# zhen6618/EPRecon

Hardware: AMD Instinct MI355X
Metric: fragments_per_sec (higher is better)
Workload: dtype f32

## Files before the change

### eprecon_amd/_lib.py

```python
import ctypes
import os

import torch

_HERE = os.path.dirname(os.path.abspath(__file__))
LIB_PATH = os.environ.get("EPRECON_LIB_PATH") or os.path.join(_HERE, "libeprecon_hip.so")

_c = ctypes
_vp, _i, _i64, _f, _sz = _c.c_void_p, _c.c_int, _c.c_int64, _c.c_float, _c.c_size_t

SIGNATURES = {
    "eprecon_abi_version": (_i, []),
    "eprecon_build_arch": (_c.c_char_p, []),
    "eprecon_back_project_workspace_bytes": (_sz, [_i64, _i, _i, _i, _i, _i, _i]),
    "eprecon_back_project_async": (_i, [_vp, _i64, _vp, _i, _f, _vp, _i, _vp, _i, _i, _i, _i, _i, _i,
                                        _vp, _vp, _vp, _vp, _vp, _vp, _vp, _vp, _sz, _vp]),
    "eprecon_back_project_call_async": (_i, [_vp, _vp]),
    "eprecon_back_project_call": (_i, [_vp, _i, _vp, _vp]),
    "eprecon_back_project_prepare_levels_async": (_i, [_vp, _i, _vp]),
    "eprecon_back_project_workspace_maps_offset": (_sz, [_i64, _i]),
    "eprecon_bp_levels": (_i, []),
    "eprecon_init_glue": (_i, []),
    "eprecon_profile_gather_kernel": (_c.c_char_p, []),
    "eprecon_hash_capacity": (_c.c_uint32, [_i64]),
# ... 72 lines not shown
    "eprecon_devoxelize_gate_tail_async": (_i, [_vp, _i, _vp, _vp, _i64, _i, _vp, _i, _i, _vp, _i, _vp, _i, _vp, _i, _vp, _i, _vp, _i,
                                                _i, _vp]),
    "eprecon_fbv_union_workspace_bytes": (_sz, [_i]),
    "eprecon_fbv_union_async": (_i, [_vp, _vp, _i64, _i, _vp, _vp, _i64, _i, _i, _i, _i, _i, _vp, _vp, _vp, _vp, _vp,
                                     _vp, _vp, _sz, _vp]),
    "eprecon_map_set_fragment": (_i, [_vp, _i]),
    "eprecon_map_stamps_async": (_i, [_vp, _vp, _vp, _i, _c.c_int32, _vp]),
    "eprecon_map_select_boundary_async": (_i, [_vp, _vp, _i, _i, _i, _vp, _vp]),
    "eprecon_map_pack_boundary_async": (_i, [_vp, _vp, _i64, _vp]),
    "eprecon_map_merge_boundary": (_i, [_vp, _vp, _i64, _vp, _i, _vp, _vp]),
    "eprecon_map_create": (_i, [_i, _c.POINTER(_vp)]),
    "eprecon_map_destroy": (_i, [_vp]),
    "eprecon_map_reset": (_i, [_vp]),
    "eprecon_map_size": (_i64, [_vp]),
    "eprecon_map_channels": (_i, [_vp]),
    "eprecon_map_export_async": (_i, [_vp, _vp, _vp, _vp]),
    "eprecon_map_import_async": (_i, [_vp, _vp, _vp, _i64, _vp]),
    "eprecon_map_crop_union": (_i, [_vp, _vp, _vp, _i64, _i, _i, _i, _i, _vp, _vp, _vp, _vp, _vp, _vp]),
    "eprecon_map_gather_async": (_i, [_vp, _vp, _i64, _i, _i, _f, _vp, _i, _vp]),
    "eprecon_map_update_async": (_i, [_vp, _vp, _i64, _vp, _i, _vp]),
    "eprecon_map_target_fuse": (_i, [_vp, _vp, _vp, _i, _vp, _vp, _i64, _vp, _vp]),
    "eprecon_gather_rows_async": (_i, [_vp, _i, _vp, _i64, _i, _f, _vp, _i, _vp]),
    "eprecon_tsdf_integrate_async": (_i, [_vp, _vp, _vp, _vp, _f, _vp, _i, _i, _i, _vp, _vp, _f, _f, _i, _vp, _vp]),
    "eprecon_gt_crop_async": (_i, [_vp, _vp]),
    "eprecon_label_volumes_workspace_bytes": (_sz, [_i64, _i64]),
    "eprecon_label_volumes": (_i, [_vp, _vp, _vp, _vp, _i64, _vp, _c.c_double, _vp, _vp, _vp, _vp, _vp, _sz, _vp]),
    "eprecon_label_fill_workspace_bytes": (_sz, [_i, _i, _i]),
    "eprecon_label_fill_async": (_i, [_vp, _vp, _vp, _vp, _sz, _vp]),
    "eprecon_marching_cubes_table": (_i, [_vp]),
    "eprecon_marching_cubes_workspace_bytes": (_sz, [_i, _i, _i]),
    "eprecon_marching_cubes_count": (_i, [_vp, _i, _i, _i, _f, _vp, _vp, _sz, _vp]),
    "eprecon_marching_cubes_emit_async": (_i, [_vp, _i, _i, _i, _f, _vp, _vp, _vp, _vp, _vp, _vp, _vp, _vp, _vp]),
    "eprecon_marching_cubes_count_masked": (_i, [_vp, _vp, _i, _i, _i, _f, _vp, _vp, _sz, _vp]),
    "eprecon_marching_cubes_emit_masked_async": (_i, [_vp, _vp, _i, _i, _i, _f, _vp, _vp, _vp, _vp, _vp, _vp, _vp, _vp, _vp]),
    "eprecon_render_depth_workspace_bytes": (_sz, [_i64]),
    "eprecon_render_depth_async": (_i, [_vp, _i64, _vp, _i64, _vp, _i, _i, _i, _f, _f, _f, _i, _vp, _i64, _vp, _sz, _vp]),
    "eprecon_render_visibility_workspace_bytes": (_sz, [_i64]),
    "eprecon_render_visibility_async": (_i, [_vp, _i64, _vp, _i64, _vp, _i, _i, _i, _f, _f, _f, _i, _vp, _i64, _vp, _sz, _vp]),
    "eprecon_render_resolve_async": (_i, [_vp, _vp, _i64, _vp, _i64, _vp, _i, _i, _i, _f, _vp, _vp, _vp, _vp, _c.c_int32, _vp, _vp,
                                          _c.c_int32, _vp, _vp, _c.c_double, _i, _i, _i, _vp, _vp]),
    "eprecon_depth_metrics_workspace_bytes": (_sz, [_i]),
    "eprecon_depth_metrics_async": (_i, [_vp, _vp, _i, _i64, _vp, _vp, _sz, _vp]),
    "eprecon_point_bounds_async": (_i, [_vp, _i64, _vp, _vp, _vp]),
    "eprecon_voxel_down_sample_workspace_bytes": (_sz, [_i64, _i64]),
    "eprecon_voxel_down_sample": (_i, [_vp, _i64, _vp, _c.c_double, _vp, _vp, _vp, _i64, _vp, _sz, _vp]),
    "eprecon_nn_search_workspace_bytes": (_sz, [_i64, _i64]),
    "eprecon_nn_search_async": (_i, [_vp, _i64, _vp, _i64, _vp, _c.c_double, _vp, _vp, _vp, _vp, _sz, _vp]),
    "eprecon_label_transfer_workspace_bytes": (_sz, [_vp, _i64]),
    "eprecon_label_bricks_async": (_i, [_vp, _vp, _vp, _i, _vp, _vp, _vp]),
    "eprecon_label_transfer_async": (_i, [_vp, _vp, _vp, _vp, _vp, _c.c_double, _vp, _i, _vp, _i64, _i, _vp, _vp, _vp, _vp, _vp, _sz,
                                          _vp]),
    "eprecon_instance_vote_async": (_i, [_vp, _vp, _i64, _i, _i, _vp, _vp, _vp, _sz, _vp]),
    "eprecon_pair_count_async": (_i, [_vp, _vp, _i64, _i, _i, _vp, _vp, _vp]),
    "eprecon_voxel_pair_count_async": (_i, [_vp, _vp, _vp, _vp, _vp, _vp, _vp, _c.c_double, _c.c_double, _f, _vp, _vp, _i, _i, _vp,
                                            _vp, _vp]),
    "eprecon_nearest_voxel_async": (_i, [_vp, _c.c_uint32, _vp, _i64, _vp, _i64, _i, _vp, _vp]),
    "eprecon_upsample2x_nhwc_async": (_i, [_vp, _vp, _i, _i, _i, _i, _vp]),
    "eprecon_decoder_keys_async": (_i, [_vp, _i, _vp, _i, _vp, _vp, _vp, _i64, _i, _vp, _vp, _vp]),
    "eprecon_decoder_query_side_async": (_i, [_vp, _vp]),
    "eprecon_panoptic_stats_async": (_i, [_vp, _i64, _vp, _vp, _i, _i64, _vp, _vp, _vp, _vp]),
    "eprecon_panoptic_assign_async": (_i, [_vp, _vp, _vp, _i64, _vp, _vp]),
    "eprecon_masked_attention_workspace_bytes": (_sz, [_i64, _i, _i, _i]),
    "eprecon_masked_attention_async": (_i, [_vp, _i, _i, _vp, _i, _vp, _i, _i64, _vp, _i, _vp, _i64, _i, _i, _i, _f, _vp, _vp, _sz, _vp]),
    "eprecon_profile_enable": (_i, [_i]),
    "eprecon_profile_gather_ms": (_f, []),
    "eprecon_profile_conv_arm": (_i, [_i, _i, _i, _i64]),
    "eprecon_profile_conv_ms": (_f, [_c.POINTER(_i64), _c.POINTER(_c.c_char_p)]),
    "eprecon_profile_conv_pairs": (_i64, []),
    "eprecon_mlp4x_supported": (_i, [_i, _i]),
    "eprecon_spvcnn_forward_workspace_bytes": (_sz, [_vp]),
    "eprecon_spvcnn_forward_async": (_i, [_vp, _vp]),
    "eprecon_spvcnn_geometry_workspace_bytes": (_sz, [_i64, _i64, _i64]),
    "eprecon_spvcnn_geometry_async": (_i, [_vp, _vp]),
    "eprecon_gru_stage_finish_workspace_bytes": (_sz, [_i64, _i64, _i64]),
    "eprecon_gru_stage_finish_async": (_i, [_vp, _vp]),
    "eprecon_bn2d_views_chunks": (_i, [_i64, _i]),
    "eprecon_bn2d_views_workspace_bytes": (_sz, [_i, _i64, _i]),
    "eprecon_bn2d_views_stats_async": (_i, [_vp, _i, _i64, _i, _vp, _vp, _f, _vp, _vp, _sz, _vp]),
    "eprecon_bn2d_views_apply_async": (_i, [_vp, _i, _i64, _i, _vp, _i, _vp, _vp, _vp]),
    "eprecon_dwconv2d_nhwc_async": (_i, [_vp, _i, _i, _i, _i, _vp, _i, _i, _vp, _i, _i, _vp, _vp]),
    "eprecon_mlp4x_async": (_i, [_vp, _vp]),
    "eprecon_profile_conv_executed_pairs": (_i64, []),
    "eprecon_profile_last_conv_kernel": (_c.c_char_p, []),
    "eprecon_profile_mark_async": (_i, [_i, _vp]),
    "eprecon_conv_desc_workspace_bytes": (_sz, [_vp]),
    "eprecon_sparsify_workspace_bytes": (_sz, [_i64]),
    "eprecon_sparsify_async": (_i, [_vp, _i, _f, _vp, _vp, _vp, _i, _vp, _i, _i, _i, _i64, _i, _vp, _vp, _vp, _vp, _vp, _vp, _vp,
                                    _sz, _vp]),
    "eprecon_grid_rank_async": (_i, [_vp, _i64, _i, _i, _i, _i, _vp, _vp]),
    "eprecon_conv_pack_weight_floats": (_sz, [_i, _i, _i]),
    "eprecon_conv_pack_weight_async": (_i, [_vp, _i, _i, _i, _vp, _vp]),
    "eprecon_conv_pack_weight16_floats": (_sz, [_i, _i, _i]),
    "eprecon_conv_pack_weight16_async": (_i, [_vp, _i, _i, _i, _vp, _vp]),
    "eprecon_conv_pack_many_async": (_i, [_vp, _i, _vp]),
    "eprecon_nchw_to_nhwc_async": (_i, [_vp, _vp, _i, _i, _i, _vp]),
    "eprecon_views_to_rows_async": (_i, [_vp, _vp]),
    "eprecon_prepare_views_async": (_i, [_vp, _i, _i, _i, _i, _i, _vp, _i, _vp, _i, _i, _i, _i, _vp, _vp]),
    "eprecon_depth_to_metres_async": (_i, [_vp, _i64, _f, _vp, _vp]),
    "eprecon_grad_sqsum_async": (_i, [_vp, _vp, _i, _vp, _vp]),
    "eprecon_grad_norm_finish_async": (_i, [_vp, _i, _f, _vp, _vp]),
    "eprecon_adam_update_async": (_i, [_vp, _vp, _i, _vp, _f, _f, _f, _f, _f, _vp, _f, _vp, _vp]),
}

VIEWS_TILE_H, VIEWS_MAX_KSIZE = 16, 9

EPRECON_OK, EPRECON_EMPTY = 0, 1
ABI_VERSION = 1


class EpreconError(RuntimeError):
    pass


_lib = None


def load():
    global _lib
    if _lib is not None:
        return _lib
    if not os.path.exists(LIB_PATH):
        raise EpreconError(
            f"{LIB_PATH} not found: build it with `python -m eprecon_amd.build` "
            "(hipcc --offload-arch=gfx950). eprecon_amd has no CPU fallback.")
    lib = ctypes.CDLL(LIB_PATH)
    for name, (res, args) in SIGNATURES.items():
        fn = getattr(lib, name)
        fn.restype = res
        fn.argtypes = args
    if lib.eprecon_abi_version() != ABI_VERSION:
        raise EpreconError("libeprecon_hip.so ABI version mismatch; rebuild")
    _lib = lib
    return lib


def check(rc, what):
    if rc == EPRECON_OK:
        return True
    if rc == EPRECON_EMPTY:
        return False
    if rc <= -1000:
        raise EpreconError(f"{what}: HIP error {-(rc + 1000)}")
    raise EpreconError(f"{what}: error {rc} "
                       "(-1 bad argument, -2 workspace too small, -3 unsupported size)")


def ptr(t):
    return None if t is None else t.data_ptr()


_raw_stream = getattr(torch._C, "_cuda_getCurrentRawStream", None)
_raw_device = getattr(torch._C, "_cuda_getDevice", None)


def current_stream():
    if _raw_stream is not None and _raw_device is not None:
        return _raw_stream(_raw_device()) or None
    return torch.cuda.current_stream().cuda_stream or None


class ViewsDesc(ctypes.Structure):
    _fields_ = [("src", (ctypes.c_void_p * 16) * 3), ("dst", ctypes.c_void_p * 3), ("channels", ctypes.c_int32 * 3),
                ("hw", ctypes.c_int32 * 3), ("levels", ctypes.c_int32), ("n_views", ctypes.c_int32)]


class BpCall(ctypes.Structure):
# ... 169 lines not shown
        if len(_DEFERRED) > _DEFERRED_MAX:
            evicted = _DEFERRED.pop(0)
    if evicted is not None:
        count_host_read()
        verify_deferred([evicted], evicted[0].to(torch.int32).tolist())


def requeue_deferred(items):
    if items:
        with _DEFERRED_LOCK:
            _DEFERRED[:0] = items


def take_deferred(stream="current"):
    st = current_stream() if stream == "current" else stream
    with _DEFERRED_LOCK:
        out = [it for it in _DEFERRED if stream is None or it[3] == st]
        _DEFERRED[:] = [it for it in _DEFERRED if not (stream is None or it[3] == st)]
    return out


def verify_deferred(items, host_values):
    for (_, expected, what, *_rest), got in zip(items, host_values):
        if int(got) != expected:
            raise EpreconError(f"{what}: expected {expected}, the device reports {int(got)} (EPRECON_ERR_ARG)")


def read_counts(counts):
    count_host_read()
    pending = take_deferred()
    flat = counts.reshape(-1)
    if pending:
        host = torch.cat([flat] + [t.reshape(1).to(flat.dtype) for t, *_ in pending]).tolist()
        verify_deferred(pending, host[flat.numel():])
        return host[:flat.numel()]
    return flat.tolist()


class PinnedRead:

    def __init__(self, counts):
        self._pending = take_deferred()
        flat = counts.reshape(-1)
        self._n = flat.numel()
        src = flat if not self._pending else torch.cat([flat] + [t.reshape(1).to(flat.dtype) for t, *_ in self._pending])
        self._pinned = torch.empty(src.numel(), dtype=src.dtype, pin_memory=True)
        self._pinned.copy_(src, non_blocking=True)
        self._event = torch.cuda.Event()
        self._event.record()

    def result(self):
        count_host_read()
        self._event.synchronize()
        host = self._pinned.tolist()
        if self._pending:
            pending, self._pending = self._pending, []
            verify_deferred(pending, host[self._n:])
        return host[:self._n]

    def __del__(self):
        try:
            requeue_deferred(self._pending)
        except Exception:
            pass


def drain_deferred():
    pending = take_deferred()
    if pending:
        count_host_read()
        verify_deferred(pending, torch.cat([t.reshape(1).to(torch.int32) for t, *_ in pending]).tolist())


HOST_READS = 0


def count_host_read(n=1):
    global HOST_READS
    HOST_READS += n


def last_conv_kernel():
    return load().eprecon_profile_last_conv_kernel().decode()
```

### eprecon_amd/csrc/sparse_conv_direct.hip

```cpp
#include "sparse_conv_direct_select.hpp"

namespace epconv {
int launch_direct16_ct1(const ConvParams &p, hipStream_t st);
int launch_direct16_ct2(const ConvParams &p, hipStream_t st);
int launch_direct16_ct3(const ConvParams &p, hipStream_t st);
int launch_direct16_ct4(const ConvParams &p, hipStream_t st);

bool direct16_ok(const ConvParams &p)
{
    if (switch_off("EPRECON_CONV_DIRECT")) return false;
    const bool pointwise = p.K == 1 && !p.nbr;
    if (!pointwise && ((p.K != 27 && p.K != 9) || !p.nbr)) return false;
    if (!p.wq16 || (reinterpret_cast<uintptr_t>(p.wq16) & 15) != 0) return false;
    if (p.Cout > 64 || p.accumulate) return false;
    if (p.ld_x % 4 != 0 || (reinterpret_cast<uintptr_t>(p.x) & 15) != 0 || (p.Cin % 4 != 0 && p.ld_x < ((p.Cin + 3) & ~3))) return false;
    if (p.x_bytes <= 0 || p.x_bytes >= 0x7fffffffll || (int64_t)p.ld_x * 4 >= (1 << 24) || p.x_bytes / ((int64_t)p.ld_x * 4) >= (1 << 24))
        return false;
    return true;
}

int direct16_partial_block_rows(const ConvParams &p) { return persist_shape_ok(p) ? kJobRows : kDirectRows; }
size_t direct16_workspace_bytes(const ConvParams &p) { return persist_shape_ok(p) ? kPersistCtrBytes : 0; }

int launch_direct16(const ConvParams &p, hipStream_t st)
{
    switch ((p.Cout + 15) / 16) {
        case 1: return launch_direct16_ct1(p, st);
        case 2: return launch_direct16_ct2(p, st);
        case 3: return launch_direct16_ct3(p, st);
        default: return launch_direct16_ct4(p, st);
    }
}

}
```

### eprecon_amd/csrc/sparse_conv_direct_device.hpp

```cpp
#pragma once
#include "sparse_conv_direct_select.hpp"

namespace epconv {
namespace {

#ifndef EP_DIRECT_ABL
#define EP_DIRECT_ABL 0
#endif

__device__ __forceinline__ float relu_nc(float x)
{
    float r;
    asm("v_max_f32 %0, 0, %1" : "=v"(r) : "v"(x));
    return r;
}
__device__ __forceinline__ float relu_sel(float x, unsigned mask)
{
    const unsigned r = __float_as_uint(relu_nc(x)), b = __float_as_uint(x);
    return __uint_as_float((r & mask) | (b & ~mask));
}

typedef __bf16 bf16x8 __attribute__((ext_vector_type(8)));
typedef __bf16 bf16x2 __attribute__((ext_vector_type(2)));
typedef short s16x4 __attribute__((ext_vector_type(4)));
typedef float f32x2 __attribute__((ext_vector_type(2)));
struct BfQuad { unsigned hi[2], lo[2]; };
__device__ __forceinline__ BfQuad bf_split(const float4 &v)
{
    const unsigned b0 = __float_as_uint(v.x), b1 = __float_as_uint(v.y), b2 = __float_as_uint(v.z), b3 = __float_as_uint(v.w);
    BfQuad r;
    r.hi[0] = __builtin_amdgcn_perm(b1, b0, 0x07060302u);
    r.hi[1] = __builtin_amdgcn_perm(b3, b2, 0x07060302u);
    const f32x2 r01 = {v.x - __uint_as_float(b0 & 0xffff0000u), v.y - __uint_as_float(b1 & 0xffff0000u)};
    const f32x2 r23 = {v.z - __uint_as_float(b2 & 0xffff0000u), v.w - __uint_as_float(b3 & 0xffff0000u)};
    r.lo[0] = __builtin_bit_cast(unsigned, __builtin_convertvector(r01, bf16x2));
    r.lo[1] = __builtin_bit_cast(unsigned, __builtin_convertvector(r23, bf16x2));
    return r;
}
__device__ __forceinline__ f32x4 bf_mfma32(const unsigned (&a0)[2], const unsigned (&a1)[2], const unsigned (&b0)[2],
                                           const unsigned (&b1)[2], f32x4 acc)
{
    union { bf16x8 v; unsigned u[4]; } a, b;
    a.u[0] = a0[0]; a.u[1] = a0[1]; a.u[2] = a1[0]; a.u[3] = a1[1];
    b.u[0] = b0[0]; b.u[1] = b0[1]; b.u[2] = b1[0]; b.u[3] = b1[1];
    return __builtin_amdgcn_mfma_f32_16x16x32_bf16(a.v, b.v, acc, 0, 0, 0);
}
__device__ __forceinline__ f32x4 bf_mfma16(const unsigned (&a0)[2], const unsigned (&b0)[2], f32x4 acc)
{
    union { s16x4 v; unsigned u[2]; } a, b;
    a.u[0] = a0[0]; a.u[1] = a0[1];
    b.u[0] = b0[0]; b.u[1] = b0[1];
    return __builtin_amdgcn_mfma_f32_16x16x16bf16_1k(a.v, b.v, acc, 0, 0, 0);
}

template <int CT, bool PERWAVE = false>
__device__ __forceinline__ void direct_epilogue(const ConvParams &p, f32x4 (&acc)[kRT][CT], int row0, float *sStat, int block = 0)
{
    constexpr int RT = kRT, NR = 4 * kRT;
    const int tid = threadIdx.x;
    const int lane = tid & 63, wave = PERWAVE ? 0 : tid >> 6;
    const int l16 = lane & 15, q = lane >> 4;
    int orow[NR];
#pragma unroll
    for (int rt = 0; rt < RT; ++rt)
#pragma unroll
        for (int j = 0; j < 4; ++j) {
            const int row = row0 + wave * 16 * RT + 16 * rt + 4 * q + j;
            orow[4 * rt + j] = row < p.n_out ? row : -1;
        }
    float v[CT][NR];
    bool colok[CT];
#pragma unroll
    for (int t = 0; t < CT; ++t) {
        const int col = 16 * t + l16;
        colok[t] = col < p.Cout;
        const float b = (p.bias && colok[t]) ? p.bias[col] : 0.0f;
        const float rs = (p.res_scale && colok[t]) ? p.res_scale[col] : 1.0f;
        const float rb = (p.res_scale && colok[t]) ? p.res_shift[col] : 0.0f;
#pragma unroll
        for (int r = 0; r < NR; ++r) {
            float val = 0.0f;
            if (colok[t] && orow[r] >= 0) {
                val = acc[r >> 2][t][r & 3] + b;
                if (p.relu) val = fmaxf(val, 0.0f);
                if (p.res) {
                    float rv = p.res[(size_t)orow[r] * p.ld_res + col];
                    if (p.res_scale) {
                        rv = fmaf(rv, rs, rb);
                        if (p.res_relu) rv = fmaxf(rv, 0.0f);
                    }
                    val += rv;
                }
            }
            v[t][r] = val;
        }
    }
    if (p.ln) {
        const float inv_c = 1.0f / (float)p.Cout;
#pragma unroll
        for (int r = 0; r < NR; ++r) {
            float sum = 0.0f;
#pragma unroll
            for (int t = 0; t < CT; ++t) sum += v[t][r];
#pragma unroll
            for (int m = 8; m > 0; m >>= 1) sum += __shfl_xor(sum, m);
            const float mean = sum * inv_c;
            float sq = 0.0f;
#pragma unroll
            for (int t = 0; t < CT; ++t) {
                const float d = colok[t] ? v[t][r] - mean : 0.0f;
                v[t][r] = d;
                sq = fmaf(d, d, sq);
            }
#pragma unroll
            for (int m = 8; m > 0; m >>= 1) sq += __shfl_xor(sq, m);
            const float inv = 1.0f / sqrtf(sq * inv_c + p.ln_eps);
#pragma unroll
            for (int t = 0; t < CT; ++t) {
                const int col = 16 * t + l16;
                float y = fmaf(v[t][r] * inv, (p.ln_gamma && colok[t]) ? p.ln_gamma[col] : 1.0f, (p.ln_beta && colok[t]) ? p.ln_beta[col] : 0.0f);
                if (p.ln_post_relu) y = fmaxf(y, 0.0f);
                v[t][r] = y;
            }
        }
    }
#pragma unroll
    for (int t = 0; t < CT; ++t)
#pragma unroll
        for (int r = 0; r < NR; ++r)
            if (colok[t] && orow[r] >= 0) p.out[(size_t)orow[r] * p.ld_out + 16 * t + l16] = v[t][r];
    if (p.bn_partial || p.bn_acc) {
#pragma unroll
        for (int t = 0; t < CT; ++t) {
            float n = 0.0f, sum = 0.0f;
#pragma unroll
            for (int r = 0; r < NR; ++r)
                if (orow[r] >= 0) { n += 1.0f; sum += v[t][r]; }
            float mean = n > 0.0f ? sum / n : 0.0f, m2 = 0.0f;
#pragma unroll
            for (int r = 0; r < NR; ++r)
                if (orow[r] >= 0) { const float d = v[t][r] - mean; m2 = fmaf(d, d, m2); }
#pragma unroll
            for (int m = 16; m < 64; m <<= 1) {
                const float on = __shfl_xor(n, m), om = __shfl_xor(mean, m), oq = __shfl_xor(m2, m);
                const bool lower = (lane & m) == 0;
                float a_n = lower ? n : on, a_mean = lower ? mean : om, a_m2 = lower ? m2 : oq;
                chan_merge(a_n, a_mean, a_m2, lower ? on : n, lower ? om : mean, lower ? oq : m2);
                n = a_n; mean = a_mean; m2 = a_m2;
            }
            if constexpr (PERWAVE) {
                if (q == 0 && colok[t]) {
                    if (p.bn_partial) bn_partial_store(p, block, 16 * t + l16, n, mean, m2);
                    if (p.bn_acc) bn_acc_publish(p, 16 * t + l16, block, block == 0, n, mean, m2);
                }
                continue;
            }
            if (q == 0) {
                float *d = sStat + (wave * 3) * 16 * CT + 16 * t + l16;
                d[0] = n; d[16 * CT] = mean; d[2 * 16 * CT] = m2;
            }
        }
        if constexpr (PERWAVE) return;
        __syncthreads();
        if (tid < 16 * CT && tid < p.Cout) {
            float a_n = 0.0f, a_mean = 0.0f, a_m2 = 0.0f;
#pragma unroll
            for (int w = 0; w < kWaves; ++w)
                chan_merge(a_n, a_mean, a_m2, sStat[(w * 3) * 16 * CT + tid], sStat[(w * 3 + 1) * 16 * CT + tid], sStat[(w * 3 + 2) * 16 * CT + tid]);
            if (p.bn_partial) bn_partial_store(p, (int)blockIdx.x, tid, a_n, a_mean, a_m2);
            if (p.bn_acc) bn_acc_publish(p, tid, (int)blockIdx.x, blockIdx.x == 0, a_n, a_mean, a_m2);
        }
    }
}

__device__ __forceinline__ void tail_to_tile(const f32x4 (&acct)[kRT][2], f32x4 (&dst)[kRT], int lane)
{
    const int l16 = lane & 15, q = lane >> 4;
    const int src = 4 * q + (l16 & 3);
#pragma unroll
    for (int rt = 0; rt < kRT; ++rt)
#pragma unroll
        for (int j = 0; j < 4; ++j) {
            float v0 = acct[rt][0][j], v1 = acct[rt][1][j];
            v0 += __shfl_xor(v0, 16); v1 += __shfl_xor(v1, 16);
            v0 += __shfl_xor(v0, 32); v1 += __shfl_xor(v1, 32);
            const float t0 = __shfl(v0, src), t1 = __shfl(v1, src);
            dst[rt][j] = l16 < 4 ? t0 : (l16 < 8 ? t1 : 0.0f);
        }
}

constexpr int kMapLoads = 14;
__device__ __forceinline__ unsigned stage_map(const ConvParams &p, int row0, int *sNbr, int *sFlag, int tid)
{
    static_assert(kDirectRows == 128 && kRT == 2 && kWaves == 4, "the pass -> (offset, row half) arithmetic below");
    const int total = p.K * kDirectRows;
    const int lane = tid & 63, wave = tid >> 6;
    int jv[kMapLoads];
#pragma unroll
    for (int it = 0; it < kMapLoads; ++it) {
        const int e = tid + it * 256;
        const int k = e >> 7, row = row0 + (e & 127);
        int j = -1;
        if (e < total && row < p.n_out) j = p.nbr ? p.nbr[(size_t)k * p.n_out + row] : row;
        jv[it] = j;
    }
#pragma unroll
    for (int it = 0; it < kMapLoads; ++it) {
        const int e = tid + it * 256;
        if (e < total) sNbr[e] = jv[it];
        const unsigned long long b = __ballot(jv[it] >= 0);
        const int k = 2 * it + (wave >> 1);
        if (lane < 2 && k < p.K) sFlag[k * kWaves + 2 * (wave & 1) + lane] = (lane ? (unsigned)(b >> 32) : (unsigned)b) != 0u;
    }
    __syncthreads();
    const bool mine = lane < p.K && sFlag[lane * kWaves + wave] != 0;
    return (unsigned)__builtin_amdgcn_readfirstlane((int)(unsigned)__ballot(mine));
}

struct LiveCursor {
    unsigned rest;
    int k, part;
    __device__ __forceinline__ explicit LiveCursor(unsigned mask) : rest(mask & (mask - 1u)), k(__builtin_ctz(mask)), part(0) {}
    __device__ __forceinline__ void next(int parts)
    {
        if (part + 1 < parts) ++part;
        else if (rest) { k = __builtin_ctz(rest); rest &= rest - 1u; part = 0; }
    }
};

#ifndef EP_MIX_EXTRA
#define EP_MIX_EXTRA 1
#endif

}
}
```

### eprecon_amd/csrc/sparse_conv_direct_launch.hpp

```cpp
#pragma once
#include "sparse_conv_direct_kernels.hpp"
#include "sparse_conv_direct_persist.hpp"

namespace epconv {
namespace {

template <int CT, int KCH>
int launch_form(const DirectForm &f, const ConvParams &p, dim3 grid, size_t lds, hipStream_t st)
{
    constexpr int G0 = stage_chunks(KCH), GA = alt_stage_chunks(KCH);
    if (f.persist) {
        if constexpr (KCH * (CT * 1024 - 512) <= 4864) {
            if (f.tail) return launch_persist<CT, KCH, true>(p, st);
            if constexpr (KCH * CT * 1024 <= 4864) return launch_persist<CT, KCH, false>(p, st);
        }
        return EPRECON_ERR_UNSUPPORTED;
    }
    void (*kern)(ConvParams) = nullptr;
    auto with_tail = [&](auto tail) {
        constexpr bool TAIL = decltype(tail)::value;
        if (f.bf) {
            if constexpr (!TAIL)
                kern = f.mode == 2   ? spconv_direct16_kernel<CT, KCH, false, G0, true, 2>
                       : f.mode == 1 ? spconv_direct16_kernel<CT, KCH, false, G0, true, 1>
                                     : spconv_direct16_kernel<CT, KCH, false, G0, true>;
        } else if (f.g != G0) {
            if constexpr (GA != 0) kern = spconv_direct16_kernel<CT, KCH, TAIL, GA>;
        } else if (f.mode >= 3) {
            if constexpr (G0 == KCH)
                kern = f.mode == 4 ? spconv_direct16_kernel<CT, KCH, TAIL, G0, false, 4> : spconv_direct16_kernel<CT, KCH, TAIL, G0, false, 3>;
        } else {
            kern = f.mode == 2   ? spconv_direct16_kernel<CT, KCH, TAIL, G0, false, 2>
                   : f.mode == 1 ? spconv_direct16_kernel<CT, KCH, TAIL, G0, false, 1>
                                 : spconv_direct16_kernel<CT, KCH, TAIL, G0>;
        }
    };
    if (f.tail) with_tail(std::true_type{});
    else with_tail(std::false_type{});
    if (!kern) return EPRECON_ERR_UNSUPPORTED;
    hipLaunchKernelGGL(kern, grid, dim3(256), lds, st, p);
    EP_LAUNCH_CHECK();
    return EPRECON_OK;
}

template <int CT, int KCH>
void stage_occupancy(bool tail, size_t lds, int &occ_p, int &occ_a)
{
    constexpr int G0 = stage_chunks(KCH), GA = alt_stage_chunks(KCH);
    static int occ[2][2] = {{0, 0}, {0, 0}};
    int *o = occ[tail ? 1 : 0];
    if (!o[0]) {
        const void *kp = tail ? reinterpret_cast<const void *>(spconv_direct16_kernel<CT, KCH, true, G0>)
                              : reinterpret_cast<const void *>(spconv_direct16_kernel<CT, KCH, false, G0>);
        const void *ka = tail ? reinterpret_cast<const void *>(spconv_direct16_kernel<CT, KCH, true, GA>)
                              : reinterpret_cast<const void *>(spconv_direct16_kernel<CT, KCH, false, GA>);
        int a = 0, b = 0;
        if (hipOccupancyMaxActiveBlocksPerMultiprocessor(&a, kp, 256, lds) != hipSuccess || a <= 0) a = 1;
        if (hipOccupancyMaxActiveBlocksPerMultiprocessor(&b, ka, 256, lds) != hipSuccess || b <= 0) b = a;
        o[1] = b;
        o[0] = a;
    }
    occ_p = o[0];
    occ_a = o[1];
}

template <int CT, int KCH>
int launch_k(const ConvParams &p, hipStream_t st)
{
    const size_t lds = direct_lds_bytes(p.K, CT, KCH);
    const DirectSwitches sw = direct_switches();
    int occ_p = 1, occ_a = 1;
    if constexpr (alt_stage_chunks(KCH) != 0) stage_occupancy<CT, KCH>(direct_tail(p, sw), lds, occ_p, occ_a);
    const DirectForm f = select_direct_form(p, sw, device_cus(), occ_p, occ_a);
    return launch_form<CT, KCH>(f, p, dim3((unsigned)ceil_div(p.n_out, kDirectRows)), lds, st);
}

template <int CT>
int launch_ct(const ConvParams &p, hipStream_t st)
{
    const int kch = (p.Cin + 15) / 16;
    if (kch <= 6) return pick<1, 2, 3, 4, 5, 6>(kch, [&](auto k) { return launch_k<CT, decltype(k)::value>(p, st); });
    hipLaunchKernelGGL((spconv_direct16_generic_kernel<CT>), dim3((unsigned)ceil_div(p.n_out, kDirectRows)), dim3(256),
                       direct_lds_bytes(p.K, CT, kch), st, p, kch);
    EP_LAUNCH_CHECK();
    return EPRECON_OK;
}

}
}
```

### eprecon_amd/csrc/sparse_conv_direct_select.hpp

```cpp
#pragma once
#include "common.hpp"
#include "conv_common.hpp"

namespace epconv {
namespace {
using namespace ep;

constexpr int kRT = 2;
constexpr int kPersistWaves = 8;
constexpr int kJobRows = 16 * kRT;
constexpr int kShares = 8, kCtrStride = 16;
constexpr size_t kPersistCtrBytes = (size_t)kShares * kCtrStride * sizeof(unsigned int);
constexpr size_t kLdsBytes = 160 * 1024;

#ifndef EP_STAGE_CAP
#define EP_STAGE_CAP 3
#endif
constexpr int stage_chunks(int kch) { return kch % 3 == 0 && EP_STAGE_CAP >= 3 ? 3 : (kch % 2 == 0 && EP_STAGE_CAP >= 2 ? 2 : 1); }
constexpr int alt_stage_chunks(int kch) { return kch == 6 ? 2 : (kch == 3 ? 1 : 0); }

static size_t direct_lds_bytes(int K, int ct, int kch)
{
    return (size_t)K * kDirectRows * sizeof(int) + (size_t)kWaves * 3 * 16 * ct * sizeof(float) + (size_t)2 * 16 * kch * sizeof(float) +
           (size_t)K * kWaves * sizeof(int);
}

static size_t persist_lds_bytes(const ConvParams &p)
{
    const int kch = (p.Cin + 15) / 16, ct = (p.Cout + 15) / 16;
    const bool tail = p.Cout - 16 * (ct - 1) <= 8;
    const size_t quads = (size_t)(tail ? ct - 1 : ct) * 64 + (tail ? 32 : 0);
    return (size_t)p.K * kch * quads * 16 + (size_t)kPersistWaves * p.K * kJobRows * sizeof(int) + (size_t)2 * 16 * kch * sizeof(float);
}

static int device_cus()
{
    static int n = 0;
    if (!n) {
        int dev = 0;
        hipDeviceProp_t prop;
        if (hipGetDevice(&dev) == hipSuccess && hipGetDeviceProperties(&prop, dev) == hipSuccess) n = prop.multiProcessorCount;
        if (n <= 0) n = 256;
    }
    return n;
}

struct DirectSwitches {
    bool tail8;
    bool interleave;
    bool stage_depth;
    bool bf16x3;
};
static DirectSwitches direct_switches()
{
    return {!switch_off("EPRECON_CONV_TAIL8"), !switch_off("EPRECON_CONV_INTERLEAVE"), !switch_off("EPRECON_CONV_STAGE_DEPTH"),
            switch_on("EPRECON_CONV_BF16X3")};
}

static bool direct_tail(const ConvParams &p, const DirectSwitches &sw)
{
    return p.Cout - 16 * ((p.Cout + 15) / 16 - 1) <= 8 && sw.tail8;
}

constexpr int kPersistMinRows = 8192;

static bool persist_shape_ok(const ConvParams &p)
{
    const int kch = (p.Cin + 15) / 16, ct = (p.Cout + 15) / 16;
    const bool rem8 = p.Cout - 16 * (ct - 1) <= 8;
    if (!switch_on("EPRECON_CONV_PERSIST") || kch > 6) return false;
    if (rem8 && switch_off("EPRECON_CONV_TAIL8")) return false;
    if (p.bn_partial && !p.flex_partial) return false;
    if (persist_lds_bytes(p) > kLdsBytes) return false;
    if (kch * ((rem8 ? ct - 1 : ct) * 1024 + (rem8 ? 512 : 0)) > 4864) return false;
    return p.n_out >= kPersistMinRows;
}
static bool persist_ok(const ConvParams &p)
{
    return persist_shape_ok(p) && p.ws && (reinterpret_cast<uintptr_t>(p.ws) & 3) == 0 && p.ws_bytes >= kPersistCtrBytes;
}

struct DirectForm {
    bool persist, tail, bf;
    int g, mode;
};

static DirectForm select_direct_form(const ConvParams &p, const DirectSwitches &sw, int cus_in, int occ_p, int occ_a)
{
    const int kch = (p.Cin + 15) / 16;
    DirectForm f = {false, false, false, 0, 0};
    if (kch > 6) return f;
    const int g0 = stage_chunks(kch);
    f.g = g0;
    if (persist_shape_ok(p)) {
        f.persist = true;
        f.tail = direct_tail(p, sw);
        return f;
    }
    int mode = 0;
    if (sw.interleave && (p.Cin & 3) == 0) {
        if (p.Cin - 16 * (kch - 1) > 8) mode = p.in_scale ? 2 : 1;
        else if (g0 == kch) mode = p.in_scale ? 4 : 3;
    }
    if (sw.bf16x3) {
        f.bf = true;
        f.mode = mode > 2 ? 0 : mode;
        return f;
    }
    f.tail = direct_tail(p, sw);
    if (alt_stage_chunks(kch) != 0 && sw.stage_depth && occ_a > occ_p && mode != 1 && mode != 3) {
        const int64_t wgs = (unsigned)ceil_div(p.n_out, kDirectRows), cus = cus_in;
        const double cost_p = (double)ceil_div(wgs, cus * occ_p) * occ_p;
        const double cost_a = (double)ceil_div(wgs, cus * occ_a) * occ_a * 1.06;
        if (cost_a < 0.85 * cost_p) {
            f.g = alt_stage_chunks(kch);
            return f;
        }
    }
    f.mode = mode;
    return f;
}

}
}
```

### include/eprecon_hip.h

```cpp
#ifndef EPRECON_HIP_H
#define EPRECON_HIP_H

#include <stddef.h>
#include <stdint.h>

#ifdef __cplusplus
extern "C" {
#endif

#define EPRECON_OK 0
#define EPRECON_EMPTY 1
#define EPRECON_ERR_ARG (-1)
#define EPRECON_ERR_WORKSPACE (-2)
#define EPRECON_ERR_UNSUPPORTED (-3)
#define EPRECON_ERR_HIP_BASE (-1000)

#define EPRECON_ABI_VERSION 1
int eprecon_abi_version(void);
const char *eprecon_build_arch(void);

#define EPRECON_BP_MEAN 0
#define EPRECON_BP_MEAN_DEPTH 1
#define EPRECON_BP_VARIANCE 2

#define EPRECON_LAYOUT_NCHW 0
#define EPRECON_LAYOUT_NHWC 1

size_t eprecon_back_project_workspace_bytes(int64_t n, int batch, int n_views, int channels,
                                            int height, int width, int feats_layout);

#define EPRECON_BP_COUNT 1
#define EPRECON_BP_GATHER 2
typedef struct eprecon_bp_call {
    const int32_t *coords;
    int64_t n;
    const float *origin;
    int32_t batch;
    float voxel_size;
    const float *feats;
    int32_t feats_layout;
    const float *krcam;
    int32_t n_views, channels, height, width, min_view, mode;
    float *count;
    int32_t *n_valid_dev;
    void *workspace;
    size_t workspace_bytes;
    int32_t phase;
    float *out_feats, *out_mean;
    int32_t *out_coords;
    float *out_grid;
    uint8_t *out_mask;
    int32_t *rank;
} eprecon_bp_call;

int eprecon_back_project_call_async(const eprecon_bp_call *call, void *stream);

int eprecon_back_project_call(const eprecon_bp_call *call, int min_valid_per_batch, int32_t *n_valid_host, void *stream);

int eprecon_back_project_async(const int32_t *coords, int64_t n, const float *origin, int batch,
                               float voxel_size, const float *feats, int feats_layout,
                               const float *krcam, int n_views, int channels, int height,
                               int width, int min_view, int mode, float *out_feats,
                               float *out_mean, int32_t *out_coords, float *count,
                               float *out_grid, uint8_t *out_mask, int32_t *n_valid_dev,
                               void *workspace, size_t workspace_bytes, void *stream);

int eprecon_back_project_prepare_levels_async(const eprecon_bp_call *levels, int n_levels, void *stream);
size_t eprecon_back_project_workspace_maps_offset(int64_t n, int batch);
int eprecon_bp_levels(void);

int eprecon_init_glue(void);

int eprecon_profile_enable(int on);
float eprecon_profile_gather_ms(void);
const char *eprecon_profile_gather_kernel(void);

int eprecon_profile_conv_arm(int kvol, int cin, int cout, int64_t min_rows);
float eprecon_profile_conv_ms(int64_t *rows_out, const char **kernel_out);
int64_t eprecon_profile_conv_pairs(void);
int64_t eprecon_profile_conv_executed_pairs(void);
const char *eprecon_profile_last_conv_kernel(void);
int eprecon_profile_mark_async(int id, void *stream);

int eprecon_nchw_to_nhwc_async(const float *in, float *out, int maps, int channels, int hw,
                               void *stream);
typedef struct eprecon_views_desc {
    const float *src[3][16];
    float *dst[3];
    int32_t channels[3]; int32_t hw[3];
    int32_t levels; int32_t n_views;
} eprecon_views_desc;
int eprecon_views_to_rows_async(const eprecon_views_desc *desc, void *stream);

uint32_t eprecon_hash_capacity(int64_t n);
size_t eprecon_hash_table_bytes(uint32_t capacity);
int eprecon_hash_build_async(const int32_t *coords, int64_t n, int quantum, void *table,
                             uint32_t capacity, void *stream);
int eprecon_hash_build_dn_async(const int32_t *coords, int64_t n_cap, const int32_t *n_dev, int quantum, void *table,
                                uint32_t capacity, void *stream);
int eprecon_hash_query_async(const void *table, uint32_t capacity, const int32_t *queries, int64_t m,
                             int quantum, int32_t *out_index, void *stream);
int eprecon_hash_status(const void *table, void *stream);

size_t eprecon_unique_workspace_bytes(int64_t n);
size_t eprecon_exclusive_scan_scratch_ints(int64_t n);
int eprecon_exclusive_scan_async(const int32_t *in, int64_t n, int32_t *out, int32_t *total, int32_t *scratch, void *stream);
int eprecon_unique_coords_async(const int32_t *coords, int64_t n, int quantum, void *table,
                                uint32_t capacity, int32_t *inverse, int32_t *unique_coords,
                                int32_t *n_unique_dev, void *workspace, size_t workspace_bytes,
                                void *stream);

int eprecon_unique_coords_dn_async(const int32_t *coords, int64_t n_cap, const int32_t *n_dev, int quantum, void *table,
                                   uint32_t capacity, int32_t *inverse, int32_t *unique_coords, int32_t *n_unique_dev,
                                   void *workspace, size_t workspace_bytes, void *stream);
int eprecon_unique_hierarchy_dn_async(const int32_t *coords, int64_t n_cap, const int32_t *n_dev, int levels, void *const *tables,
                                      const uint32_t *capacities, int32_t *const *inverse, int32_t *const *unique_coords,
                                      int32_t *summary, void *workspace, size_t workspace_bytes, void *stream);

int eprecon_kernel_map_self_async(const void *table, uint32_t capacity, const int32_t *coords, int64_t n, int stride, int32_t *nbr,
                                  void *stream);
int eprecon_kernel_map_async(const void *table, uint32_t capacity, const int32_t *coords, int64_t n,
                             int ksize, int stride, int32_t *nbr, void *stream);
int eprecon_transpose_map_async(const int32_t *fine_coords, int64_t n, const int32_t *parent,
                                int fine_stride, int32_t *up_map, void *stream);
int eprecon_sparse_conv_async(const float *x, int64_t n_in, int ld_x, const int32_t *nbr, int kvol,
                              int64_t n_out, const float *weight, int cin, int cout, const float *bias,
                              float *out, int ld_out, int relu, int accumulate, void *stream);
size_t eprecon_conv_bn_partial_bytes(int64_t n_out, int cout);
int eprecon_sparse_conv_fused_async(const float *x, int64_t n_in, int ld_x, const int32_t *nbr, int kvol,
                                    int64_t n_out, const float *weight, int cin, int cout,
                                    const float *bias, const float *residual, int ld_res, float *out,
                                    int ld_out, int relu, int accumulate, float *bn_partial, void *stream);
typedef struct eprecon_conv_desc {
    const float *x; int64_t n_in; int ld_x;
    const int32_t *nbr; int kvol; int64_t n_out;
    const float *weight; int cin; int cout;
    const float *bias;
    const float *residual; int ld_res;
    float *out; int ld_out;
    int relu; int accumulate;
    const float *in_scale; const float *in_shift; int in_relu;
    const float *res_scale; const float *res_shift; int res_relu;
    float *bn_partial; int bn_ld;
    int ln; const float *ln_gamma; const float *ln_beta; float ln_eps; int ln_post_relu;
    int img_h; int img_w; int img_maps;
    const int32_t *vox_rank; int grid_x; int grid_y; int grid_z;
    const float *packed_weight;
    const float *packed_weight16;
    void *workspace; size_t workspace_bytes;
    long long *bn_acc; int bn_acc_ld; int bn_acc_c0; const float *bn_gamma; const float *bn_beta;
    const long long *in_acc; int in_acc_ld; int in_acc_c0; float in_eps; float *in_affine_scratch;
} eprecon_conv_desc;
size_t eprecon_bn_acc_words(int ld);
int eprecon_conv_desc_takes_bn_acc(const eprecon_conv_desc *desc);
int eprecon_batchnorm_acc_affine_async(const long long *acc, int acc_ld, int acc_c0, int channels, float eps, float *scale_out,
                                       float *shift_out, void *stream);
int eprecon_affine_rows_acc_async(const float *x, int64_t n, int channels, int ld_x, const long long *acc, int acc_ld, int acc_c0,
                                  float eps, int relu, float *out, int ld_out, void *stream);
int eprecon_conv_desc_async(const eprecon_conv_desc *desc, void *stream);
size_t eprecon_conv_desc_workspace_bytes(const eprecon_conv_desc *desc);
int64_t eprecon_conv_desc_partial_rows(const eprecon_conv_desc *desc);
int eprecon_conv_dense3d_kind(const eprecon_conv_desc *desc);
int eprecon_batchnorm_finalize_affine_async(const float *partial, int64_t nblk, int64_t ld, int channels, const float *gamma,
                                            const float *beta, float eps, float *scale_out, float *shift_out,
// ... 442 lines not shown
```

Measured before the change: 817.7.

## Add persistent streaming kernel for pointwise sparse convolutions with double-buffered loads

Adds a persistent, grid-strided kernel for K=1 (pointwise) sparse convolutions with large Cin. It double-buffers input loads across channel-chunk groups so global fetches overlap MFMA compute, and it launches only enough workgroups to fill the device at measured occupancy. BN statistics are written per logical block instead of per blockIdx. It also extends chunk support to Cin up to 256 and adds a debug symbol query. In exchange it brings new selection heuristics and env switches, and the persistent loop lowers parallelism for mid-sized inputs.

```diff
diff --git a/eprecon_amd/_lib.py b/eprecon_amd/_lib.py
--- a/eprecon_amd/_lib.py
+++ b/eprecon_amd/_lib.py
@@ -178,6 +178,7 @@
     "eprecon_mlp4x_async": (_i, [_vp, _vp]),
     "eprecon_profile_conv_executed_pairs": (_i64, []),
     "eprecon_profile_last_conv_kernel": (_c.c_char_p, []),
+    "eprecon_profile_last_direct_symbol": (_c.c_char_p, []),
     "eprecon_profile_mark_async": (_i, [_i, _vp]),
     "eprecon_conv_desc_workspace_bytes": (_sz, [_vp]),
     "eprecon_sparsify_workspace_bytes": (_sz, [_i64]),
@@ -513,3 +514,7 @@
 
 def last_conv_kernel():
     return load().eprecon_profile_last_conv_kernel().decode()
+
+
+def last_direct_symbol():
+    return load().eprecon_profile_last_direct_symbol().decode()
diff --git a/eprecon_amd/csrc/sparse_conv_direct.hip b/eprecon_amd/csrc/sparse_conv_direct.hip
--- a/eprecon_amd/csrc/sparse_conv_direct.hip
+++ b/eprecon_amd/csrc/sparse_conv_direct.hip
@@ -22,6 +22,8 @@
 int direct16_partial_block_rows(const ConvParams &p) { return persist_shape_ok(p) ? kJobRows : kDirectRows; }
 size_t direct16_workspace_bytes(const ConvParams &p) { return persist_shape_ok(p) ? kPersistCtrBytes : 0; }
 
+const char *g_last_direct_symbol = "";
+
 int launch_direct16(const ConvParams &p, hipStream_t st)
 {
     switch ((p.Cout + 15) / 16) {
@@ -33,3 +35,5 @@
 }
 
 }
+
+extern "C" const char *eprecon_profile_last_direct_symbol(void) { return epconv::g_last_direct_symbol; }
diff --git a/eprecon_amd/csrc/sparse_conv_direct_device.hpp b/eprecon_amd/csrc/sparse_conv_direct_device.hpp
--- a/eprecon_amd/csrc/sparse_conv_direct_device.hpp
+++ b/eprecon_amd/csrc/sparse_conv_direct_device.hpp
@@ -53,7 +53,7 @@
     return __builtin_amdgcn_mfma_f32_16x16x16bf16_1k(a.v, b.v, acc, 0, 0, 0);
 }
 
-template <int CT, bool PERWAVE = false>
+template <int CT, bool PERWAVE = false, bool STRIDED = false>
 __device__ __forceinline__ void direct_epilogue(const ConvParams &p, f32x4 (&acc)[kRT][CT], int row0, float *sStat, int block = 0)
 {
     constexpr int RT = kRT, NR = 4 * kRT;
@@ -163,12 +163,13 @@
         if constexpr (PERWAVE) return;
         __syncthreads();
         if (tid < 16 * CT && tid < p.Cout) {
+            const int srow = STRIDED ? block : (int)blockIdx.x;
             float a_n = 0.0f, a_mean = 0.0f, a_m2 = 0.0f;
 #pragma unroll
             for (int w = 0; w < kWaves; ++w)
                 chan_merge(a_n, a_mean, a_m2, sStat[(w * 3) * 16 * CT + tid], sStat[(w * 3 + 1) * 16 * CT + tid], sStat[(w * 3 + 2) * 16 * CT + tid]);
-            if (p.bn_partial) bn_partial_store(p, (int)blockIdx.x, tid, a_n, a_mean, a_m2);
-            if (p.bn_acc) bn_acc_publish(p, tid, (int)blockIdx.x, blockIdx.x == 0, a_n, a_mean, a_m2);
+            if (p.bn_partial) bn_partial_store(p, srow, tid, a_n, a_mean, a_m2);
+            if (p.bn_acc) bn_acc_publish(p, tid, srow, srow == 0, a_n, a_mean, a_m2);
         }
     }
 }
diff --git a/eprecon_amd/csrc/sparse_conv_direct_k1.hpp b/eprecon_amd/csrc/sparse_conv_direct_k1.hpp
--- /dev/null
+++ b/eprecon_amd/csrc/sparse_conv_direct_k1.hpp
@@ -0,0 +1,202 @@
+#pragma once
+#include "sparse_conv_direct_device.hpp"
+
+namespace epconv {
+namespace {
+
+template <int CT, bool TAIL, int D>
+__global__ __launch_bounds__(256) void spconv_direct16_k1_kernel(ConvParams p, int kch, int nblk)
+{
+    extern __shared__ __attribute__((aligned(16))) char smem[];
+    constexpr int RT = kRT, ROWS = kDirectRows;
+    constexpr int CTM = TAIL ? CT - 1 : CT;
+    constexpr int CTA = CTM > 0 ? CTM : 1;
+    constexpr int NS = CTM == 1 ? 2 : 1;
+    const int cpad = 16 * kch;
+    const int wquads = kch * (CT * 64 + (TAIL ? 32 : 0));
+    float4 *sW = reinterpret_cast<float4 *>(smem);
+    float *sStat = reinterpret_cast<float *>(sW + wquads);
+    float *sAff = sStat + kWaves * 3 * 16 * CT;
+    const float4 *sWt = sW + kch * CT * 64;
+    const int tid = threadIdx.x;
+    const int lane = tid & 63, wave = tid >> 6;
+    const int l16 = lane & 15, q = lane >> 4;
+    const int ng = (kch + D - 1) / D;
+
+    const __amdgpu_buffer_rsrc_t xrsrc = __builtin_amdgcn_make_buffer_rsrc(const_cast<float *>(p.x), 0, (int)p.x_bytes, 0x00020000);
+    const unsigned row_bytes = (unsigned)p.ld_x * 4u, oob = (unsigned)p.x_bytes;
+    const int last_c = p.Cin - 16 * (kch - 1);
+    const bool tail8 = last_c <= 8;
+    const unsigned cq = 16u * (unsigned)q;
+    const unsigned cq_last = tail8 ? 8u * (unsigned)q : cq;
+    const bool last_ok = (tail8 ? 2 : 4) * q < last_c;
+    const unsigned relu_mask = p.in_relu ? 0xffffffffu : 0u;
+
+    struct Cursor {
+        int blk, g;
+        __device__ __forceinline__ void next(int ng, int step)
+        {
+            if (++g == ng) { g = 0; blk += step; }
+        }
+    };
+    struct Stage {
+        float4 a[D][RT];
+    };
+    auto fetch = [&](const Cursor &c, Stage &g) {
+        unsigned rowsel[RT];
+#pragma unroll
+        for (int rt = 0; rt < RT; ++rt) {
+            const int row = c.blk * ROWS + wave * 16 * RT + 16 * rt + l16;
+            rowsel[rt] = (c.blk < nblk && row < p.n_out) ? __umul24((unsigned)row, row_bytes) : oob;
+        }
+#pragma unroll
+        for (int i = 0; i < D; ++i) {
+            const int kc = c.g * D + i;
+#pragma unroll
+            for (int rt = 0; rt < RT; ++rt) {
+                unsigned off = oob;
+                if (rowsel[rt] != oob) {
+                    if (kc < kch - 1) off = rowsel[rt] + 64u * (unsigned)kc + cq;
+                    else if (kc == kch - 1 && last_ok) off = rowsel[rt] + 64u * (unsigned)kc + cq_last;
+                }
+                const u32x4 v = __builtin_amdgcn_raw_buffer_load_b128(xrsrc, off, 0, 0);
+                g.a[i][rt] = make_float4(__uint_as_float(v.x), __uint_as_float(v.y), __uint_as_float(v.z), __uint_as_float(v.w));
+            }
+        }
+    };
+
+    f32x4 acc[NS][RT][CTA];
+    f32x4 acct[RT][2];
+    auto clear = [&]() {
+#pragma unroll
+        for (int rt = 0; rt < RT; ++rt) {
+#pragma unroll
+            for (int ns = 0; ns < NS; ++ns)
+#pragma unroll
+                for (int t = 0; t < CTA; ++t) acc[ns][rt][t] = f32x4{0.0f, 0.0f, 0.0f, 0.0f};
+            acct[rt][0] = acct[rt][1] = f32x4{0.0f, 0.0f, 0.0f, 0.0f};
+        }
+    };
+    auto consume = [&](const Cursor &c, const Stage &g) {
+        bool rok[RT];
+#pragma unroll
+        for (int rt = 0; rt < RT; ++rt) rok[rt] = c.blk * ROWS + wave * 16 * RT + 16 * rt + l16 < p.n_out;
+#pragma unroll
+        for (int i = 0; i < D; ++i) {
+            const int kc = c.g * D + i;
+            if (kc >= kch) break;
+            const bool is_last = kc == kch - 1;
+            const bool t8 = tail8 && is_last;
+            float4 b[CTA], bt[2];
+#pragma unroll
+            for (int t = 0; t < CTM; ++t) b[t] = sW[(kc * CT + t) * 64 + lane];
+            if constexpr (TAIL) {
+#pragma unroll
+                for (int cg = 0; cg < 2; ++cg) bt[cg] = sWt[kc * 32 + cg * 16 + 4 * q + (lane & 3)];
+            }
+            float4 av[RT];
+#pragma unroll
+            for (int rt = 0; rt < RT; ++rt) av[rt] = g.a[i][rt];
+            const int ca = 16 * kc + (t8 ? 2 : 4) * q;
+            const bool ragged = (p.Cin & 3) && is_last;
+            if (ragged) {
+#pragma unroll
+                for (int rt = 0; rt < RT; ++rt) {
+                    if (ca + 1 >= p.Cin) av[rt].y = 0.0f;
+                    if (ca + 2 >= p.Cin) av[rt].z = 0.0f;
+                    if (ca + 3 >= p.Cin) av[rt].w = 0.0f;
+                }
+            }
+            if (p.in_scale) {
+                const float4 sc = make_float4(sAff[ca], sAff[ca + 1], sAff[ca + 2], sAff[ca + 3]);
+                const float4 sh = make_float4(sAff[cpad + ca], sAff[cpad + ca + 1], sAff[cpad + ca + 2], sAff[cpad + ca + 3]);
+                const bool cok = is_last ? last_ok : true;
+#pragma unroll
+                for (int rt = 0; rt < RT; ++rt) {
+                    float4 x = av[rt];
+                    x.x = fmaf(x.x, sc.x, sh.x); x.y = fmaf(x.y, sc.y, sh.y); x.z = fmaf(x.z, sc.z, sh.z); x.w = fmaf(x.w, sc.w, sh.w);
+                    x.x = relu_sel(x.x, relu_mask); x.y = relu_sel(x.y, relu_mask);
+                    x.z = relu_sel(x.z, relu_mask); x.w = relu_sel(x.w, relu_mask);
+                    if (ragged) {
+                        if (ca + 1 >= p.Cin) x.y = 0.0f;
+                        if (ca + 2 >= p.Cin) x.z = 0.0f;
+                        if (ca + 3 >= p.Cin) x.w = 0.0f;
+                    }
+                    av[rt] = (rok[rt] && cok) ? x : make_float4(0.0f, 0.0f, 0.0f, 0.0f);
+                }
+            }
+#define EP_K1_STEP(comp, set)                                                                                                        \
+    do {                                                                                                                             \
+        _Pragma("unroll") for (int rt = 0; rt < RT; ++rt)                                                                            \
+            _Pragma("unroll") for (int t = 0; t < CTM; ++t)                                                                          \
+                acc[(set) % NS][rt][t] = __builtin_amdgcn_mfma_f32_16x16x4f32(av[rt].comp, b[t].comp, acc[(set) % NS][rt][t], 0, 0, 0); \
+        if constexpr (TAIL) {                                                                                                        \
+            _Pragma("unroll") for (int rt = 0; rt < RT; ++rt)                                                                        \
+                _Pragma("unroll") for (int cg = 0; cg < 2; ++cg)                                                                     \
+                    acct[rt][cg] = __builtin_amdgcn_mfma_f32_4x4x1f32(av[rt].comp, bt[cg].comp, acct[rt][cg], 0, 0, 0);              \
+        }                                                                                                                            \
+    } while (0)
+            EP_K1_STEP(x, 0);
+            EP_K1_STEP(y, 1);
+            if (!t8) {
+                EP_K1_STEP(z, 0);
+                EP_K1_STEP(w, 1);
+            }
+#undef EP_K1_STEP
+        }
+    };
+    auto finish = [&](const Cursor &c) {
+        if constexpr (NS == 2) {
+#pragma unroll
+            for (int rt = 0; rt < RT; ++rt)
+#pragma unroll
+                for (int t = 0; t < CTM; ++t) acc[0][rt][t] += acc[1][rt][t];
+        }
+        if (p.bn_partial || p.bn_acc) __syncthreads();
+        if constexpr (TAIL) {
+            f32x4 full[RT][CT];
+            f32x4 last[RT];
+            tail_to_tile(acct, last, lane);
+#pragma unroll
+            for (int rt = 0; rt < RT; ++rt) {
+#pragma unroll
+                for (int t = 0; t < CTM; ++t) full[rt][t] = acc[0][rt][t];
+                full[rt][CT - 1] = last[rt];
+            }
+            direct_epilogue<CT, false, true>(p, full, c.blk * ROWS, sStat, c.blk);
+        } else {
+            direct_epilogue<CT, false, true>(p, acc[0], c.blk * ROWS, sStat, c.blk);
+        }
+        clear();
+    };
+
+    const int step = (int)gridDim.x;
+    Cursor cf = {(int)blockIdx.x, 0}, cc = cf;
+    Stage s_c, s_n;
+    fetch(cf, s_c);
+    {
+        const float4 *wsrc = reinterpret_cast<const float4 *>(p.wq16);
+        for (int e = tid; e < wquads; e += 256) sW[e] = wsrc[e];
+        stage_in_affine<256, false>(p, sAff, cpad, tid);
+        clear();
+        __syncthreads();
+    }
+#pragma clang loop unroll(disable)
+    for (;;) {
+        cf.next(ng, step);
+        fetch(cf, s_n);
+        __builtin_amdgcn_sched_barrier(0);
+        consume(cc, s_c);
+        __builtin_amdgcn_sched_barrier(0);
+        __builtin_amdgcn_s_waitcnt(0x0f70);
+        s_c = s_n;
+        __builtin_amdgcn_sched_barrier(0);
+        if (cc.g == ng - 1) finish(cc);
+        cc.next(ng, step);
+        if (cc.blk >= nblk) break;
+        __builtin_amdgcn_sched_barrier(0);
+    }
+}
+
+}
+}
diff --git a/eprecon_amd/csrc/sparse_conv_direct_launch.hpp b/eprecon_amd/csrc/sparse_conv_direct_launch.hpp
--- a/eprecon_amd/csrc/sparse_conv_direct_launch.hpp
+++ b/eprecon_amd/csrc/sparse_conv_direct_launch.hpp
@@ -1,8 +1,10 @@
 #pragma once
+#include "sparse_conv_direct_k1.hpp"
 #include "sparse_conv_direct_kernels.hpp"
 #include "sparse_conv_direct_persist.hpp"
 
 namespace epconv {
+extern const char *g_last_direct_symbol;
 namespace {
 
 template <int CT, int KCH>
@@ -11,6 +13,7 @@
     constexpr int G0 = stage_chunks(KCH), GA = alt_stage_chunks(KCH);
     if (f.persist) {
         if constexpr (KCH * (CT * 1024 - 512) <= 4864) {
+            g_last_direct_symbol = "spconv_persist16_kernel";
             if (f.tail) return launch_persist<CT, KCH, true>(p, st);
             if constexpr (KCH * CT * 1024 <= 4864) return launch_persist<CT, KCH, false>(p, st);
         }
@@ -38,6 +41,7 @@
     if (f.tail) with_tail(std::true_type{});
     else with_tail(std::false_type{});
     if (!kern) return EPRECON_ERR_UNSUPPORTED;
+    g_last_direct_symbol = "spconv_direct16_kernel";
     hipLaunchKernelGGL(kern, grid, dim3(256), lds, st, p);
     EP_LAUNCH_CHECK();
     return EPRECON_OK;
@@ -76,10 +80,39 @@
 }
 
 template <int CT>
+int launch_k1(const DirectForm &f, const DirectSwitches &sw, const ConvParams &p, hipStream_t st)
+{
+    const int kch = (p.Cin + 15) / 16;
+    const size_t lds = k1_lds_bytes(CT, kch, f.tail);
+    void (*kern)(ConvParams, int, int) =
+        f.tail ? spconv_direct16_k1_kernel<CT, true, kK1StageChunks> : spconv_direct16_k1_kernel<CT, false, kK1StageChunks>;
+    static int occ[2][kK1MaxChunks + 1];
+    int &o = occ[f.tail ? 1 : 0][kch];
+    if (!o) {
+        int a = 0;
+        if (hipOccupancyMaxActiveBlocksPerMultiprocessor(&a, reinterpret_cast<const void *>(kern), 256, lds) != hipSuccess || a <= 0) a = 1;
+        o = a;
+    }
+    const int64_t nblk = ceil_div(p.n_out, kDirectRows);
+    int64_t wgs = (int64_t)device_cus() * o;
+    if (sw.k1_wgs > 0 && sw.k1_wgs < wgs) wgs = sw.k1_wgs;
+    g_last_direct_symbol = "spconv_direct16_k1_kernel";
+    hipLaunchKernelGGL(kern, dim3((unsigned)(nblk < wgs ? nblk : wgs)), dim3(256), lds, st, p, kch, (int)nblk);
+    EP_LAUNCH_CHECK();
+    return EPRECON_OK;
+}
+
+template <int CT>
 int launch_ct(const ConvParams &p, hipStream_t st)
 {
     const int kch = (p.Cin + 15) / 16;
+    if (p.K == 1 && !p.nbr) {
+        const DirectSwitches sw = direct_switches();
+        const DirectForm f = select_direct_form(p, sw, device_cus(), 1, 1);
+        if (f.k1) return launch_k1<CT>(f, sw, p, st);
+    }
     if (kch <= 6) return pick<1, 2, 3, 4, 5, 6>(kch, [&](auto k) { return launch_k<CT, decltype(k)::value>(p, st); });
+    g_last_direct_symbol = "spconv_direct16_generic_kernel";
     hipLaunchKernelGGL((spconv_direct16_generic_kernel<CT>), dim3((unsigned)ceil_div(p.n_out, kDirectRows)), dim3(256),
                        direct_lds_bytes(p.K, CT, kch), st, p, kch);
     EP_LAUNCH_CHECK();
diff --git a/eprecon_amd/csrc/sparse_conv_direct_select.hpp b/eprecon_amd/csrc/sparse_conv_direct_select.hpp
--- a/eprecon_amd/csrc/sparse_conv_direct_select.hpp
+++ b/eprecon_amd/csrc/sparse_conv_direct_select.hpp
@@ -50,11 +50,14 @@
     bool interleave;
     bool stage_depth;
     bool bf16x3;
+    int k1_stream;
+    int k1_wgs;
 };
 static DirectSwitches direct_switches()
 {
+    const char *wgs = getenv("EPRECON_CONV_K1_WGS"), *k1 = getenv("EPRECON_CONV_K1_STREAM");
     return {!switch_off("EPRECON_CONV_TAIL8"), !switch_off("EPRECON_CONV_INTERLEAVE"), !switch_off("EPRECON_CONV_STAGE_DEPTH"),
-            switch_on("EPRECON_CONV_BF16X3")};
+            switch_on("EPRECON_CONV_BF16X3"), k1 && k1[0] == '0' ? 0 : (k1 && k1[0] == '2' ? 2 : 1), wgs ? atoi(wgs) : 0};
 }
 
 static bool direct_tail(const ConvParams &p, const DirectSwitches &sw)
@@ -80,15 +83,39 @@
     return persist_shape_ok(p) && p.ws && (reinterpret_cast<uintptr_t>(p.ws) & 3) == 0 && p.ws_bytes >= kPersistCtrBytes;
 }
 
+constexpr int kK1MaxChunks = 16;
+constexpr int kK1StageChunks = 2;
+static size_t k1_lds_bytes(int ct, int kch, bool tail)
+{
+    return (size_t)kch * (ct * 1024 + (tail ? 512 : 0)) + (size_t)kWaves * 3 * 16 * ct * sizeof(float) + (size_t)2 * 16 * kch * sizeof(float);
+}
+constexpr int kK1StreamMinCin = 64, kK1StreamBlocksPerCu = 3;
+static bool k1_stream_ok(const ConvParams &p, const DirectSwitches &sw, int cus)
+{
+    if (p.K != 1 || p.nbr || !sw.k1_stream || sw.bf16x3 || p.in_acc || p.debug != 0) return false;
+    const int kch = (p.Cin + 15) / 16, ct = (p.Cout + 15) / 16;
+    if (kch > kK1MaxChunks || persist_shape_ok(p)) return false;
+    if (k1_lds_bytes(ct, kch, true) > dynamic_lds_limit()) return false;
+    if (sw.k1_stream == 2) return true;
+    return p.Cin >= kK1StreamMinCin && ceil_div(p.n_out, kDirectRows) > (int64_t)kK1StreamBlocksPerCu * cus;
+}
+
 struct DirectForm {
     bool persist, tail, bf;
     int g, mode;
+    bool k1;
 };
 
 static DirectForm select_direct_form(const ConvParams &p, const DirectSwitches &sw, int cus_in, int occ_p, int occ_a)
 {
     const int kch = (p.Cin + 15) / 16;
-    DirectForm f = {false, false, false, 0, 0};
+    DirectForm f = {false, false, false, 0, 0, false};
+    if (k1_stream_ok(p, sw, cus_in)) {
+        f.k1 = true;
+        f.tail = kch <= 6 && direct_tail(p, sw);
+        f.g = kK1StageChunks;
+        return f;
+    }
     if (kch > 6) return f;
     const int g0 = stage_chunks(kch);
     f.g = g0;
diff --git a/include/eprecon_hip.h b/include/eprecon_hip.h
--- a/include/eprecon_hip.h
+++ b/include/eprecon_hip.h
@@ -80,6 +80,7 @@
 int64_t eprecon_profile_conv_pairs(void);
 int64_t eprecon_profile_conv_executed_pairs(void);
 const char *eprecon_profile_last_conv_kernel(void);
+const char *eprecon_profile_last_direct_symbol(void);
 int eprecon_profile_mark_async(int id, void *stream);
 
 int eprecon_nchw_to_nhwc_async(const float *in, float *out, int maps, int channels, int hw,
```

New measurement: 821.3 (median of 6 runs). No clear change (+0.4%).
